# KohakuBlueleaf/UwUDiff

Measured on AMD Instinct MI355X. Metric: train images/sec (whole node), DiT-S/2 256^2 latent, higher is better.
Workload: dtype bf16; 1 GPU; DiT-S/2 (L12 D384 h6), 4x32x32 synthetic latents + pooled-text cond 1280, eps-MSE, AdamW lr1e-6 wd0.01 cosine; random-init weights; per_gpu_batch=768, global_batch=768, parallelism=dp1

## Files before the change

### uwudiff_amd/csrc/gemm_as.hip

```cpp
#include "gemm_shared.h"

namespace {

constexpr int AS_K = 384, AS_BN = 64, AS_STAGE = AS_BN * AS_K * 2;
constexpr int AS_NST = 3;
constexpr int AS_LDS = AS_NST * AS_STAGE + 8192;
template <typename TC, int EPI>
__global__ void __launch_bounds__(512, 2) gemm_as_kernel(const GemmArgs g) {
  extern __shared__ __attribute__((aligned(16))) char smem[];
  typedef bf16_t T;
  constexpr int FI = 2, FJ = 4, KS = AS_K / 32;
  const int tid = threadIdx.x, lane = tid & 63;
  const int wave = __builtin_amdgcn_readfirstlane(tid >> 6);
  const int fr = lane & 15, fq = lane >> 4;
  const int m0 = blockIdx.x * 256 + wave * 32;
  const T* A = static_cast<const T*>(g.A);
  const T* B = static_cast<const T*>(g.B);
  float* bias_lds = reinterpret_cast<float*>(smem + AS_NST * AS_STAGE);
  if (EPI == UWU_EPI_BIAS || EPI == UWU_EPI_BIAS_GELU)
    for (int n = tid; n < g.N; n += 512) bias_lds[n] = g.bias[n];

  uint4 af[FI][KS];
#pragma unroll
  for (int i = 0; i < FI; ++i)
#pragma unroll
    for (int s = 0; s < KS; ++s)
      af[i][s] = *reinterpret_cast<const uint4*>(A + (int64_t)(m0 + 16 * i + fr) * g.lda + 32 * s + 8 * fq);

  const int drow = 8 * wave + (lane >> 3);
  const int dc = ((lane & 7) ^ (drow >> 1) ^ (drow >> 4)) & 7;
  const T* bsrc = B + (int64_t)drow * g.ldb + 8 * dc;
  const unsigned smem_base = (unsigned)(size_t)((const __attribute__((address_space(3))) char*)smem);
  auto issue = [&](int c) {
    const T* p = bsrc + (int64_t)c * AS_BN * g.ldb;
#pragma unroll
    for (int q = 0; q < AS_K / 64; ++q)
      glds16_asm(p + 64 * q, smem_base + (unsigned)((c % AS_NST) * AS_STAGE + q * 8192 + wave * 1024));
  };
  const int nchunks = g.N / AS_BN;
  static_assert(EPI == UWU_EPI_BIAS_GELU || EPI == UWU_EPI_BIAS || EPI == UWU_EPI_DGELU, "the interleaved epilogues");
  constexpr int NS = EPI == UWU_EPI_BIAS ? 4 : 8;
  TC* const C = static_cast<TC*>(g.C);
  TC* const C2 = static_cast<TC*>(g.C2);
  const bool odd = fq & 1;
  auto pack = [](const f32x4& v) {
    bf16x4 b = {(bf16_t)v[0], (bf16_t)v[1], (bf16_t)v[2], (bf16_t)v[3]};
    return *reinterpret_cast<uint2*>(&b);
  };
  uint4 auxr[4];
  const T* const auxp = static_cast<const T*>(g.aux);
  auto aux_load = [&](int n0, int u) {
    const int i = u >> 1, jp = u & 1;
    const int m = m0 + 16 * i + fr, n = n0 + 32 * jp + (odd ? 16 + 4 * (fq - 1) : 4 * fq);
    auxr[u] = *reinterpret_cast<const uint4*>(auxp + (int64_t)m * g.ldaux + n);
  };
  auto epi_unit = [&](const f32x4 (&pa)[FI][FJ], int n0, int i, int jp) {
    f32x4 v0 = pa[i][2 * jp], v1 = pa[i][2 * jp + 1];
    typedef unsigned su32x2 __attribute__((ext_vector_type(2)));
    typedef unsigned su32x4 __attribute__((ext_vector_type(4)));
    if constexpr (EPI == UWU_EPI_DGELU) {
      const uint4 a = auxr[2 * i + jp];
      const su32x2 sx = __builtin_amdgcn_permlane16_swap(a.x, a.z, false, false);
      const su32x2 sy = __builtin_amdgcn_permlane16_swap(a.y, a.w, false, false);
      const uint2 r0 = {sx[0], sy[0]}, r1 = {sx[1], sy[1]};
      const bf16x4 u0 = *reinterpret_cast<const bf16x4*>(&r0), u1 = *reinterpret_cast<const bf16x4*>(&r1);
      v0 = v0 * dgelu_tanh_f4(f32x4{(float)u0[0], (float)u0[1], (float)u0[2], (float)u0[3]});
      v1 = v1 * dgelu_tanh_f4(f32x4{(float)u1[0], (float)u1[1], (float)u1[2], (float)u1[3]});
    } else {
      const float* bl = bias_lds + n0 + 32 * jp + 4 * fq;
      v0 = v0 + *reinterpret_cast<const f32x4*>(bl);
      v1 = v1 + *reinterpret_cast<const f32x4*>(bl + 16);
    }
    const int m = m0 + 16 * i + fr;
    const int n = n0 + 32 * jp + (odd ? 16 + 4 * (fq - 1) : 4 * fq);
    auto exchange_store = [&](TC* dst, const f32x4& x0, const f32x4& x1, bool stream_out) {
      const uint2 p0 = pack(x0), p1 = pack(x1);
      const su32x2 sx = __builtin_amdgcn_permlane16_swap(p0.x, p1.x, false, false);
      const su32x2 sy = __builtin_amdgcn_permlane16_swap(p0.y, p1.y, false, false);
      const su32x4 o = su32x4{sx[0], sy[0], sx[1], sy[1]};
      su32x4* ptr = reinterpret_cast<su32x4*>(dst + (int64_t)m * g.ldc + n);
      if (stream_out) __builtin_nontemporal_store(o, ptr);
      else *ptr = o;
    };
    if constexpr (EPI == UWU_EPI_BIAS_GELU) {
      exchange_store(C, v0, v1, true);
      exchange_store(C2, gelu_tanh_f4(v0), gelu_tanh_f4(v1), false);
    } else {
      exchange_store(C, v0, v1, false);
    }
  };
  f32x4 prev[FI][FJ];
#pragma unroll
  for (int i = 0; i < FI; ++i)
#pragma unroll
    for (int j = 0; j < FJ; ++j) prev[i][j] = f32x4{0.f, 0.f, 0.f, 0.f};
  issue(0);
  issue(1);
  for (int c = 0; c < nchunks; ++c) {
    if (c == 0) asm volatile("s_waitcnt vmcnt(6) lgkmcnt(0)" ::: "memory");
    else if (c <= 2 || c + 1 >= nchunks) asm volatile("s_waitcnt vmcnt(0)" ::: "memory");
    else asm volatile("s_waitcnt vmcnt(%0)" ::"n"(2 * NS + 6) : "memory");
    __builtin_amdgcn_s_barrier();
    if (c + 2 < nchunks) issue(c + 2);
    const char* lb = smem + (c % AS_NST) * AS_STAGE;
    f32x4 acc[FI][FJ];
#pragma unroll
    for (int i = 0; i < FI; ++i)
#pragma unroll
      for (int j = 0; j < FJ; ++j) acc[i][j] = f32x4{0.f, 0.f, 0.f, 0.f};
    constexpr int NBF = EPI == UWU_EPI_DGELU ? 1 : 2;
    uint4 bf[NBF][FJ];
    auto frags = [&](uint4 (&dst)[FJ], int s) {
#pragma unroll
      for (int j = 0; j < FJ; ++j)
        dst[j] = *reinterpret_cast<const uint4*>(lb + (s >> 1) * 8192 + swz(16 * j + fr, 4 * (s & 1) + fq));
    };
    if constexpr (NBF == 2) frags(bf[0], 0);
#pragma unroll
    for (int s = 0; s < KS; ++s) {
      if constexpr (NBF == 2) {
        if (s + 1 < KS) frags(bf[(s + 1) & 1], s + 1);
      } else {
        frags(bf[0], s);
      }
#pragma unroll
      for (int i = 0; i < FI; ++i)
#pragma unroll
        for (int j = 0; j < FJ; ++j) mma_frag<T>(bf[s & (NBF - 1)][j], af[i][s], acc[i][j]);
      if (s % 3 == 1) {
        if (c > 0) epi_unit(prev, (c - 1) * AS_BN, (s / 3) >> 1, (s / 3) & 1);
        if constexpr (EPI == UWU_EPI_DGELU) aux_load(c * AS_BN, s / 3);
      }
    }
#pragma unroll
    for (int i = 0; i < FI; ++i)
#pragma unroll
      for (int j = 0; j < FJ; ++j) prev[i][j] = acc[i][j];
  }
#pragma unroll
  for (int u = 0; u < 4; ++u) epi_unit(prev, (nchunks - 1) * AS_BN, u >> 1, u & 1);
}

}

bool uwu_gemm_use_as(const GemmArgs& g, int out_bytes) {
  static UwuEnv on("UWU_GEMM_AS");
  if (on.get().is('0')) return false;
  return g.K == AS_K && g.M % 256 == 0 && g.M >= 256 * 256 && g.N % AS_BN == 0 && g.N <= 2048 && g.N >= 1024 && out_bytes == 2 &&
         g.lda % 8 == 0 &&
         g.ldb % 8 == 0 && g.ldc % 8 == 0 && (((uintptr_t)g.A | (uintptr_t)g.B | (uintptr_t)g.C | (uintptr_t)g.C2) & 15) == 0;
}
bool uwu_gemm_use_as_bias() {
  static UwuEnv on("UWU_GEMM_AS_BIAS");
  return !on.get().is('0');
}


template <typename TC, int EPI>
int uwu_launch_gemm_as(GemmArgs g, hipStream_t st) {
  g.wide = 1;
  return gemm_launch<gemm_as_kernel<TC, EPI>>("gemm_as", AS_LDS, dim3(g.M / 256), 512, st, gemm_prof(g, false, sizeof(TC)), g);
}

template int uwu_launch_gemm_as<bf16_t, UWU_EPI_BIAS>(GemmArgs, hipStream_t);
template int uwu_launch_gemm_as<bf16_t, UWU_EPI_BIAS_GELU>(GemmArgs, hipStream_t);
template int uwu_launch_gemm_as<bf16_t, UWU_EPI_DGELU>(GemmArgs, hipStream_t);
```

### uwudiff_amd/csrc/gemm_shared.h

```cpp
#pragma once
#include <stdlib.h>

#include <atomic>
#include <type_traits>

#include "common.h"

#define RETURN_IF(...)             \
  do {                             \
    const int rc_ = (__VA_ARGS__); \
    if (rc_ != UWU_OK) return rc_; \
  } while (0)

extern std::atomic<const char*> g_uwu_gemm_last_kernel;

struct GemmArgs {
  const void* A;
  const void* B;
  void* C;
  void* C2;
  const float* bias;
  const void* aux;
  int M, N, K, lda, ldb, ldc, ldaux, epi, tiles_m, tiles_n, k_tiles_per_split, wide;
  int xs, nloc, part_m;
  int aux16;
  int cH, cW, cC, cHo, cWo, cS;
  const void* zero;
  void* q8;
  void* q8t;
  const float* q_scale;
  float* q_amax;
  int ldq, ldqt;
};

namespace {

constexpr int BM = 128, BN = 128;
constexpr int ROW_BYTES = 128;
constexpr int TILE_BYTES = 128 * ROW_BYTES;

template <typename T> struct GT;
template <> struct GT<bf16_t> { static constexpr int EPC = 8; static constexpr int BK = 64; };
template <> struct GT<float> { static constexpr int EPC = 4; static constexpr int BK = 32; };

__device__ __forceinline__ int swz(int row, int chunk) {
  return row * ROW_BYTES + (((chunk ^ (row >> 1) ^ (row >> 4)) & 7) << 4);
}

typedef unsigned gu32x4 __attribute__((ext_vector_type(4)));
__device__ __forceinline__ uint4 lds_read128_asm(const char* p) {
  gu32x4 v;
  const unsigned a = (unsigned)(size_t)((const __attribute__((address_space(3))) char*)p);
  asm volatile("ds_read_b128 %0, %1" : "=v"(v) : "v"(a) : "memory");
  return uint4{v[0], v[1], v[2], v[3]};
}

template <typename T, bool TRANS>
struct Stager {
  uint4 r[4];

  __device__ __forceinline__ void load(const T* __restrict__ base, int ld, int row0, int k0, int nrows, int K,
                                       int tid) {
    constexpr int EPC = GT<T>::EPC;
    if constexpr (!TRANS) {
      const int c = tid & 7, rr = tid >> 3;
      const int kk = k0 + c * EPC;
#pragma unroll
      for (int p = 0; p < 4; ++p) {
        const int grow = row0 + rr + 32 * p;
        if (grow < nrows && kk < K)
          r[p] = *reinterpret_cast<const uint4*>(base + (int64_t)grow * ld + kk);
        else
          r[p] = uint4{0, 0, 0, 0};
      }
    } else if constexpr (sizeof(T) == 2) {
      const int xg = tid & 15, kg = tid >> 4;
      const int x = row0 + 8 * xg;
#pragma unroll
      for (int kr = 0; kr < 4; ++kr) {
        const int k = k0 + 4 * kg + kr;
        if (k < K && x < nrows)
          r[kr] = *reinterpret_cast<const uint4*>(base + (int64_t)k * ld + x);
        else
          r[kr] = uint4{0, 0, 0, 0};
      }
    } else {
      const int xg = tid & 31, kg = tid >> 5;
      const int x = row0 + 4 * xg;
#pragma unroll
      for (int kr = 0; kr < 4; ++kr) {
        const int k = k0 + 4 * kg + kr;
        if (k < K && x < nrows)
          r[kr] = *reinterpret_cast<const uint4*>(base + (int64_t)k * ld + x);
        else
          r[kr] = uint4{0, 0, 0, 0};
      }
    }
  }

  __device__ __forceinline__ void store(char* __restrict__ lds, int tid) const {
    if constexpr (!TRANS) {
      const int c = tid & 7, rr = tid >> 3;
#pragma unroll
      for (int p = 0; p < 4; ++p) *reinterpret_cast<uint4*>(lds + swz(rr + 32 * p, c)) = r[p];
    } else if constexpr (sizeof(T) == 2) {
      const int xg = tid & 15, kg = tid >> 4;
      const unsigned* w0 = reinterpret_cast<const unsigned*>(&r[0]);
      const unsigned* w1 = reinterpret_cast<const unsigned*>(&r[1]);
      const unsigned* w2 = reinterpret_cast<const unsigned*>(&r[2]);
      const unsigned* w3 = reinterpret_cast<const unsigned*>(&r[3]);
#pragma unroll
      for (int xi = 0; xi < 8; ++xi) {
        const int row = 8 * xg + xi;
        const unsigned sel = (xi & 1) ? 0x07060302u : 0x05040100u;
        uint2 o;
        o.x = __builtin_amdgcn_perm(w1[xi >> 1], w0[xi >> 1], sel);
        o.y = __builtin_amdgcn_perm(w3[xi >> 1], w2[xi >> 1], sel);
        *reinterpret_cast<uint2*>(lds + swz(row, kg >> 1) + 8 * (kg & 1)) = o;
      }
    } else {
      const int xg = tid & 31, kg = tid >> 5;
      const unsigned* w0 = reinterpret_cast<const unsigned*>(&r[0]);
      const unsigned* w1 = reinterpret_cast<const unsigned*>(&r[1]);
      const unsigned* w2 = reinterpret_cast<const unsigned*>(&r[2]);
      const unsigned* w3 = reinterpret_cast<const unsigned*>(&r[3]);
#pragma unroll
      for (int xi = 0; xi < 4; ++xi) {
        const int row = 4 * xg + xi;
        *reinterpret_cast<uint4*>(lds + swz(row, kg)) = uint4{w0[xi], w1[xi], w2[xi], w3[xi]};
      }
    }
  }
};

template <typename T>
__device__ __forceinline__ void glds_tile(const T* __restrict__ base, int ld, int row0, int k0, int nrows,
                                          char* __restrict__ lds_tile, int tid) {
  constexpr int EPC = GT<T>::EPC;
  const int wave = tid >> 6, lane = tid & 63;
#pragma unroll
  for (int g = 0; g < 4; ++g) {
    const int grp = wave + 4 * g;
    const int row = 8 * grp + (lane >> 3);
    const int c = ((lane & 7) ^ (row >> 1) ^ (row >> 4)) & 7;
    int grow = row0 + row;
    if (grow >= nrows) grow = nrows - 1;
    const T* src = base + (int64_t)grow * ld + k0 + c * EPC;
    __builtin_amdgcn_global_load_lds((const __attribute__((address_space(1))) void*)src,
                                     (__attribute__((address_space(3))) void*)(lds_tile + grp * 1024), 16, 0, 0);
  }
}

template <typename T>
__device__ __forceinline__ void mma_frag(const uint4& a, const uint4& b, f32x4& c) {
  if constexpr (sizeof(T) == 2) {
    c = __builtin_amdgcn_mfma_f32_16x16x32_bf16(*reinterpret_cast<const bf16x8*>(&a),
                                                *reinterpret_cast<const bf16x8*>(&b), c, 0, 0, 0);
  } else {
    const float* af = reinterpret_cast<const float*>(&a);
    const float* bf = reinterpret_cast<const float*>(&b);
#pragma unroll
    for (int e = 0; e < 4; ++e) c = __builtin_amdgcn_mfma_f32_16x16x4f32(af[e], bf[e], c, 0, 0, 0);
  }
}



__device__ __forceinline__ void divmod24(int n, int d, float rcp, int& q, int& r) {
  q = (int)((float)n * rcp);
  r = n - q * d;
  if (r < 0) { r += d; --q; }
  if (r >= d) { r -= d; ++q; }
}

template <typename T, int FI, int FJ>
struct EpiPre {
  static constexpr int PD = FI < 4 ? FI : 4;
  typedef typename std::conditional<sizeof(T) == 2, uint2, f32x4>::type AuxRaw;
  f32x4 bias[FJ];
  AuxRaw aux[PD][FJ];
};
template <typename T, int FI, int FJ>
__device__ __forceinline__ void epi_load_aux_row(const GemmArgs& g, int m_w, int n_w, int fr, int fq, int i,
                                                 typename EpiPre<T, FI, FJ>::AuxRaw (&dst)[FJ]) {
  typedef typename EpiPre<T, FI, FJ>::AuxRaw AuxRaw;
  const T* aux = static_cast<const T*>(g.aux);
  const int m = m_w + 16 * i + fr;
  if constexpr (sizeof(T) == 2 && FJ % 2 == 0) {
    if (g.aux16) {
      const bool odd = fq & 1;
#pragma unroll
      for (int jp = 0; jp < FJ / 2; ++jp) {
        const int nb = n_w + 32 * jp;
        const int n = odd ? nb + 16 + 4 * (fq - 1) : nb + 4 * fq;
        uint4 v = {0u, 0u, 0u, 0u};
        if (m < g.M && n < g.N) v = *reinterpret_cast<const uint4*>(aux + (int64_t)m * g.ldaux + n);
        dst[2 * jp] = AuxRaw{v.x, v.y};
        dst[2 * jp + 1] = AuxRaw{v.z, v.w};
      }
      return;
    }
  }
#pragma unroll
  for (int j = 0; j < FJ; ++j) {
    const int n = n_w + 16 * j + 4 * fq;
    if (m < g.M && n < g.N) dst[j] = *reinterpret_cast<const AuxRaw*>(aux + (int64_t)m * g.ldaux + n);
    else dst[j] = AuxRaw{};
  }
}
template <typename T, int FI, int FJ, int EPI>
__device__ __forceinline__ void epi_prefetch(EpiPre<T, FI, FJ>& pre, const GemmArgs& g, int m_w, int n_w, int fr,
                                             int fq) {
  const int epi = EPI >= 0 ? EPI : g.epi;
  const bool has_bias = epi == UWU_EPI_BIAS || epi == UWU_EPI_BIAS_GELU || epi == UWU_EPI_BIAS_SILU;
#pragma unroll
  for (int j = 0; j < FJ; ++j) {
    const int n = n_w + 16 * j + 4 * fq;
    pre.bias[j] = (has_bias && n < g.N) ? load4(g.bias + n) : f32x4{0.f, 0.f, 0.f, 0.f};
  }
  if (epi == UWU_EPI_DGELU) {
#pragma unroll
    for (int i = 0; i < EpiPre<T, FI, FJ>::PD; ++i) epi_load_aux_row<T, FI, FJ>(g, m_w, n_w, fr, fq, i, pre.aux[i]);
  }
}

template <typename T, typename TC, int FI, int FJ, int EPI = -1>
__device__ __forceinline__ void epilogue_tile(f32x4 (&acc)[FI][FJ], EpiPre<T, FI, FJ>& pre, const GemmArgs& g, int m_w,
                                              int n_w, int fr, int fq, float* cs_lds, int wm, int wn, int cs_t = -1,
                                              f32x4* cs_out = nullptr) {
  TC* C = static_cast<TC*>(g.C);
  TC* C2 = static_cast<TC*>(g.C2);
  const int epi = EPI >= 0 ? EPI : g.epi;
  const bool has_bias = epi == UWU_EPI_BIAS || epi == UWU_EPI_BIAS_GELU || epi == UWU_EPI_BIAS_SILU;
  const bool two = epi == UWU_EPI_BIAS_GELU || epi == UWU_EPI_BIAS_SILU;
  const bool dgelu = epi == UWU_EPI_DGELU;
  constexpr int PD = EpiPre<T, FI, FJ>::PD;
  typedef typename EpiPre<T, FI, FJ>::AuxRaw AuxRaw;
  auto aux_f32 = [](const AuxRaw& r) {
    if constexpr (sizeof(T) == 2) {
      const bf16x4 b = *reinterpret_cast<const bf16x4*>(&r);
      return f32x4{(float)b[0], (float)b[1], (float)b[2], (float)b[3]};
    } else {
      return r;
    }
  };

  auto finish = [&](f32x4 v, const f32x4& b, const AuxRaw& a, f32x4& second) {
    if (has_bias) v = v + b;
    if (dgelu) {
      v = v * dgelu_tanh_f4(aux_f32(a));
    }
    if (epi == UWU_EPI_BIAS_GELU) {
      second = gelu_tanh_f4(v);
    } else if (epi == UWU_EPI_BIAS_SILU) {
#pragma unroll
      for (int e = 0; e < 4; ++e) second[e] = silu_f(v[e]);
    }
    return v;
  };
  float* colsum = dgelu ? reinterpret_cast<float*>(g.C2) : nullptr;
  f32x4 csum[FJ];
#pragma unroll
  for (int j = 0; j < FJ; ++j) csum[j] = f32x4{0.f, 0.f, 0.f, 0.f};
  auto add_cs = [&](f32x4& acc_, const f32x4& v) { acc_ = acc_ + v; };
  auto flush_cs = [&]() {
    if (!colsum) return;
    constexpr int BNT = 2 * 16 * FJ;
    __syncthreads();
#pragma unroll
    for (int j = 0; j < FJ; ++j) {
      f32x4 v = csum[j];
#pragma unroll
      for (int e = 0; e < 4; ++e) v[e] = row16_sum(v[e]);
      if (fr == 0) store4(cs_lds + wm * BNT + wn * 16 * FJ + 16 * j + 4 * fq, v);
    }
    __syncthreads();
    const int t = cs_t >= 0 ? cs_t : (int)threadIdx.x, n = n_w - wn * 16 * FJ + t;
    if (t < BNT && n < g.N) atomicAdd(colsum + n, cs_lds[t] + cs_lds[BNT + t]);
  };
  const bool wide = sizeof(TC) == 2 && g.wide;
  const bool odd = fq & 1;
  auto pack = [](const f32x4& v) {
    bf16x4 b = {(bf16_t)v[0], (bf16_t)v[1], (bf16_t)v[2], (bf16_t)v[3]};
    return *reinterpret_cast<uint2*>(&b);
  };
#pragma unroll
  for (int i = 0; i < FI; ++i) {
    const int m = m_w + 16 * i + fr;
    const bool mok = m < g.M;
    AuxRaw(&arow)[FJ] = pre.aux[i % PD];
    if constexpr (sizeof(T) == 2 && FJ % 2 == 0) {
      if (dgelu && g.aux16) {
#pragma unroll
        for (int jp = 0; jp < FJ / 2; ++jp) {
          typedef unsigned su32x2 __attribute__((ext_vector_type(2)));
          const su32x2 sx = __builtin_amdgcn_permlane16_swap(arow[2 * jp].x, arow[2 * jp + 1].x, false, false);
          const su32x2 sy = __builtin_amdgcn_permlane16_swap(arow[2 * jp].y, arow[2 * jp + 1].y, false, false);
          arow[2 * jp] = AuxRaw{sx[0], sy[0]};
          arow[2 * jp + 1] = AuxRaw{sx[1], sy[1]};
        }
      }
    }
    f32x4 v[FJ], sec[FJ];
#pragma unroll
    for (int j = 0; j < FJ; ++j) {
      const int n = n_w + 16 * j + 4 * fq;
      sec[j] = f32x4{0.f, 0.f, 0.f, 0.f};
      v[j] = (mok && n < g.N) ? finish(acc[i][j], pre.bias[j], arow[j], sec[j]) : acc[i][j];
      if (colsum && mok && n < g.N) add_cs(csum[j], v[j]);
    }
    if (dgelu && i + PD < FI) epi_load_aux_row<T, FI, FJ>(g, m_w, n_w, fr, fq, i + PD, arow);
    if (wide) {
      if constexpr (sizeof(TC) == 2) {
#pragma unroll
        for (int jp = 0; jp < FJ / 2; ++jp) {
          const int nb = n_w + 32 * jp;
          auto exchange_store = [&](TC* dst, const f32x4& x0, const f32x4& x1, bool stream_out = false) {
            const uint2 p0 = pack(x0), p1 = pack(x1);
            typedef unsigned su32x2 __attribute__((ext_vector_type(2)));
            const su32x2 sx = __builtin_amdgcn_permlane16_swap(p0.x, p1.x, false, false);
            const su32x2 sy = __builtin_amdgcn_permlane16_swap(p0.y, p1.y, false, false);
            const int n = odd ? nb + 16 + 4 * (fq - 1) : nb + 4 * fq;
            if (mok && n < g.N) {
              typedef unsigned su32x4 __attribute__((ext_vector_type(4)));
              const su32x4 o = su32x4{sx[0], sy[0], sx[1], sy[1]};
              su32x4* ptr = reinterpret_cast<su32x4*>(dst + (int64_t)m * g.ldc + n);
              if (stream_out) __builtin_nontemporal_store(o, ptr);
              else *ptr = o;
            }
          };
          exchange_store(C, v[2 * jp], v[2 * jp + 1], epi == UWU_EPI_BIAS_GELU);
          if (two) exchange_store(C2, sec[2 * jp], sec[2 * jp + 1], false);
        }
      }
    } else {
#pragma unroll
      for (int j = 0; j < FJ; ++j) {
        const int n = n_w + 16 * j + 4 * fq;
        if (!mok || n >= g.N) continue;
        store4(C + (int64_t)m * g.ldc + n, v[j]);
        if (two) store4(C2 + (int64_t)m * g.ldc + n, sec[j]);
      }
    }
  }
  if (cs_out) {
#pragma unroll
    for (int j = 0; j < FJ; ++j) cs_out[j] = cs_out[j] + csum[j];
  } else {
    flush_cs();
  }
}

constexpr int R_ROWB = 64;
constexpr int R_BSUB = 32 * 256;

__device__ __forceinline__ int r_gsw(int row) { return (0 - (row >> 2)) & 3; }
__device__ __forceinline__ int r_swz(int row, int chunk) { return row * R_ROWB + (((chunk ^ r_gsw(row)) & 3) << 4); }
template <int OFF>
__device__ __forceinline__ uint4 r_read128(unsigned addr) {
  gu32x4 v;
  asm volatile("ds_read_b128 %0, %1 offset:%2" : "=v"(v) : "v"(addr), "n"(OFF) : "memory");
  return uint4{v[0], v[1], v[2], v[3]};
}
template <int N>
__device__ __forceinline__ void r_wait_vm() {
  asm volatile("s_waitcnt vmcnt(%0)" ::"n"(N) : "memory");
}
__device__ __forceinline__ void glds16_asm(const void* gsrc, unsigned lds_dst ) {
  unsigned keep;
  asm volatile("s_mov_b32 %0, m0\n\ts_mov_b32 m0, %2\n\ts_nop 0\n\tglobal_load_lds_dwordx4 %1, off\n\ts_mov_b32 m0, %0"
               : "=&s"(keep)
               : "v"(gsrc), "s"(lds_dst)
               : "memory");
}
template <int H>
using IC = std::integral_constant<int, H>;
__device__ __forceinline__ int p8_swz(int row, int chunk) { return row * ROW_BYTES + (((chunk ^ (row >> 1)) & 7) << 4); }

template <int OFF>
__device__ __forceinline__ uint2 t_read_tr(unsigned addr) {
  typedef unsigned tu32x2 __attribute__((ext_vector_type(2)));
  tu32x2 v;
  asm volatile("ds_read_b64_tr_b16 %0, %1 offset:%2" : "=v"(v) : "v"(addr), "n"(OFF) : "memory");
  return uint2{v[0], v[1]};
}
__device__ __forceinline__ unsigned tr_lane_base(int lane, int t, int xb8) {
  const int tg = lane >> 4, tq = (lane >> 2) & 3, tp = lane & 3;
  const int krow = 8 * tg + 4 * t + tq;
  const int f = (tq << 2) | ((2 * tg + t) & 3);
  return (unsigned)(256 * krow + 16 * ((xb8 + (tp >> 1)) ^ f) + 8 * (tp & 1));
}

static int gemm_tag(const GemmArgs& g, bool tb, bool acc) {
  if (acc) return UWU_PROF_GEMM_WGRAD;
  if (g.epi == UWU_EPI_BIAS_GELU) return UWU_PROF_GEMM_FC1_GELU;
  if (g.epi == UWU_EPI_DGELU) return UWU_PROF_GEMM_FC2_DGELU;
  return tb ? UWU_PROF_GEMM_DGRAD : UWU_PROF_GEMM_FWD;
}
static double gemm_bytes(const GemmArgs& g, int es, int esc) {
  double b = ((double)g.M * g.K + (double)g.N * g.K) * es + (double)g.M * g.N * esc;
  if (g.epi == UWU_EPI_BIAS_GELU || g.epi == UWU_EPI_BIAS_SILU) b += (double)g.M * g.N * esc;
  if (g.epi == UWU_EPI_DGELU) b += (double)g.M * g.N * es;
  return b;
}

template <auto KERN>
int gemm_lds_optin(const char* name, int lds) {
  static unsigned char done[UWU_MAX_DEV];
  if (uwu_func_lds(reinterpret_cast<const void*>(KERN), lds, done)) return UWU_OK;
  uwu_set_error("%s: the device cannot give a workgroup %d bytes of LDS", name, lds);
  return UWU_ELAUNCH;
}
struct GemmProf {
  int tag, kind;
  double flops, bytes;
};
static GemmProf gemm_prof(const GemmArgs& g, bool tb, int esc) {
  return {gemm_tag(g, tb, false), 0, 2.0 * g.M * g.N * g.K, gemm_bytes(g, 2, esc)};
}
template <auto KERN, typename... Args>
int gemm_launch(const char* name, int lds, dim3 grid, int block, hipStream_t st, const GemmProf& p, const Args&... args) {
  RETURN_IF(gemm_lds_optin<KERN>(name, lds));
  g_uwu_gemm_last_kernel.store(name, std::memory_order_relaxed);
  UwuProfScope prof(st);
  hipLaunchKernelGGL(KERN, grid, dim3(block), lds, st, args...);
  prof.done(p.tag, p.kind, p.flops, p.bytes);
  UWU_LAUNCH_CHECK(name);
  return UWU_OK;
}

}

bool uwu_gemm_use_as(const GemmArgs& g, int out_bytes);
bool uwu_gemm_use_as_bias();
template <typename TC, int EPI> int uwu_launch_gemm_as(GemmArgs g, hipStream_t st);
int uwu_conv3x3_args(GemmArgs& g, int B, int H, int W, int C, int stride);
int uwu_gemm_pick_tr(const GemmArgs& g);
template <int FI, int FJ, bool CONVW = false> int uwu_launch_gemm_tr(GemmArgs g, void* scratch, size_t scratch_bytes, hipStream_t st);
void uwu_launch_splitk_reduce(const float* part, float* C, int M, int N, int ldc, int split, hipStream_t st);
int uwu_launch_gemm_p8(const GemmArgs& g, bool tb, hipStream_t st);
int uwu_p8_cus();
bool uwu_gemm_p8_ok(const GemmArgs& g, bool tb);
int uwu_launch_gemm_p8n(const GemmArgs& g, bool tb, hipStream_t st);
bool uwu_gemm_p8n_ok(const GemmArgs& g, bool tb);
bool uwu_gemm_p8f_ok(const GemmArgs& g);
int uwu_launch_gemm_p8f(GemmArgs g, int fmt_a, const float* sa, const float* sb, hipStream_t st);
int uwu_gemm_p8f_split(int tiles, int steps);
bool uwu_gemm_p8f_part_ok(const GemmArgs& g);
int uwu_launch_gemm_p8f_part(GemmArgs& g, int fmt_a, const float* sa, const float* sb, void* scratch, hipStream_t st);
```

Before: 17860 images/s.

## Split B-tile loads across two wave groups in the DGELU AS GEMM

```diff
diff --git a/uwudiff_amd/csrc/gemm_as.hip b/uwudiff_amd/csrc/gemm_as.hip
--- a/uwudiff_amd/csrc/gemm_as.hip
+++ b/uwudiff_amd/csrc/gemm_as.hip
@@ -5,7 +5,7 @@
 constexpr int AS_K = 384, AS_BN = 64, AS_STAGE = AS_BN * AS_K * 2;
 constexpr int AS_NST = 3;
 constexpr int AS_LDS = AS_NST * AS_STAGE + 8192;
-template <typename TC, int EPI>
+template <typename TC, int EPI, bool GRP>
 __global__ void __launch_bounds__(512, 2) gemm_as_kernel(const GemmArgs g) {
   extern __shared__ __attribute__((aligned(16))) char smem[];
   typedef bf16_t T;
@@ -31,11 +31,16 @@
   const int dc = ((lane & 7) ^ (drow >> 1) ^ (drow >> 4)) & 7;
   const T* bsrc = B + (int64_t)drow * g.ldb + 8 * dc;
   const unsigned smem_base = (unsigned)(size_t)((const __attribute__((address_space(3))) char*)smem);
+  const unsigned boff = (unsigned)(drow * g.ldb + 8 * dc) * 2;
   auto issue = [&](int c) {
     const T* p = bsrc + (int64_t)c * AS_BN * g.ldb;
-#pragma unroll
-    for (int q = 0; q < AS_K / 64; ++q)
-      glds16_asm(p + 64 * q, smem_base + (unsigned)((c % AS_NST) * AS_STAGE + q * 8192 + wave * 1024));
+    const T* ps = B + (int64_t)c * AS_BN * g.ldb;
+#pragma unroll
+    for (int q = 0; q < AS_K / 64; ++q) {
+      const unsigned dst = smem_base + (unsigned)((c % AS_NST) * AS_STAGE + q * 8192 + wave * 1024);
+      if constexpr (GRP) glds16_asm_s(ps + 64 * q, boff, dst);
+      else glds16_asm(p + 64 * q, dst);
+    }
   };
   const int nchunks = g.N / AS_BN;
   static_assert(EPI == UWU_EPI_BIAS_GELU || EPI == UWU_EPI_BIAS || EPI == UWU_EPI_DGELU, "the interleaved epilogues");
@@ -94,14 +99,33 @@
   for (int i = 0; i < FI; ++i)
 #pragma unroll
     for (int j = 0; j < FJ; ++j) prev[i][j] = f32x4{0.f, 0.f, 0.f, 0.f};
+  const int grp = GRP ? wave >> 2 : 0;
+  auto wait_chunk = [&](int w) __attribute__((always_inline)) {
+    if (w <= 2 || w + 1 >= nchunks) asm volatile("s_waitcnt vmcnt(0)" ::: "memory");
+    else asm volatile("s_waitcnt vmcnt(%0)" ::"n"(GRP ? 3 * NS / 2 + 6 : 2 * NS + 6) : "memory");
+  };
   issue(0);
   issue(1);
+  if (GRP && grp == 1) {
+    asm volatile("s_waitcnt vmcnt(6) lgkmcnt(0)" ::: "memory");
+    __builtin_amdgcn_s_barrier();
+  }
   for (int c = 0; c < nchunks; ++c) {
-    if (c == 0) asm volatile("s_waitcnt vmcnt(6) lgkmcnt(0)" ::: "memory");
-    else if (c <= 2 || c + 1 >= nchunks) asm volatile("s_waitcnt vmcnt(0)" ::: "memory");
-    else asm volatile("s_waitcnt vmcnt(%0)" ::"n"(2 * NS + 6) : "memory");
-    __builtin_amdgcn_s_barrier();
-    if (c + 2 < nchunks) issue(c + 2);
+    if constexpr (!GRP) {
+      if (c == 0) asm volatile("s_waitcnt vmcnt(6) lgkmcnt(0)" ::: "memory");
+      else wait_chunk(c);
+      __builtin_amdgcn_s_barrier();
+      if (c + 2 < nchunks) issue(c + 2);
+    } else {
+      asm volatile("s_waitcnt lgkmcnt(0)" ::: "memory");
+      if (grp == 0) {
+        if (c == 0) asm volatile("s_waitcnt vmcnt(6)" ::: "memory");
+        else wait_chunk(c);
+      }
+      __builtin_amdgcn_s_barrier();
+      __builtin_amdgcn_sched_barrier(0);
+      if (grp == 1 && c + 2 < nchunks) issue(c + 2);
+    }
     const char* lb = smem + (c % AS_NST) * AS_STAGE;
     f32x4 acc[FI][FJ];
 #pragma unroll
@@ -123,6 +147,14 @@
       } else {
         frags(bf[0], s);
       }
+      if constexpr (GRP) {
+        if (s == KS / 2) {
+          if (grp == 1 && c + 1 < nchunks) wait_chunk(c + 1);
+          __builtin_amdgcn_s_barrier();
+          __builtin_amdgcn_sched_barrier(0);
+          if (grp == 0 && c + 2 < nchunks) issue(c + 2);
+        }
+      }
 #pragma unroll
       for (int i = 0; i < FI; ++i)
 #pragma unroll
@@ -139,6 +171,7 @@
   }
 #pragma unroll
   for (int u = 0; u < 4; ++u) epi_unit(prev, (nchunks - 1) * AS_BN, u >> 1, u & 1);
+  if (GRP && grp == 0) __builtin_amdgcn_s_barrier();
 }
 
 }
@@ -158,8 +191,12 @@
 
 template <typename TC, int EPI>
 int uwu_launch_gemm_as(GemmArgs g, hipStream_t st) {
+  static UwuEnv groups("UWU_AS_GROUPS");
   g.wide = 1;
-  return gemm_launch<gemm_as_kernel<TC, EPI>>("gemm_as", AS_LDS, dim3(g.M / 256), 512, st, gemm_prof(g, false, sizeof(TC)), g);
+  constexpr bool grouped = EPI == UWU_EPI_DGELU;
+  if (!grouped || groups.get().is('0'))
+    return gemm_launch<gemm_as_kernel<TC, EPI, false>>("gemm_as", AS_LDS, dim3(g.M / 256), 512, st, gemm_prof(g, false, sizeof(TC)), g);
+  return gemm_launch<gemm_as_kernel<TC, EPI, grouped>>("gemm_as", AS_LDS, dim3(g.M / 256), 512, st, gemm_prof(g, false, sizeof(TC)), g);
 }
 
 template int uwu_launch_gemm_as<bf16_t, UWU_EPI_BIAS>(GemmArgs, hipStream_t);
diff --git a/uwudiff_amd/csrc/gemm_shared.h b/uwudiff_amd/csrc/gemm_shared.h
--- a/uwudiff_amd/csrc/gemm_shared.h
+++ b/uwudiff_amd/csrc/gemm_shared.h
@@ -373,6 +373,13 @@
                : "v"(gsrc), "s"(lds_dst)
                : "memory");
 }
+__device__ __forceinline__ void glds16_asm_s(const void* gbase , unsigned lane_off, unsigned lds_dst ) {
+  unsigned keep;
+  asm volatile("s_mov_b32 %0, m0\n\ts_mov_b32 m0, %3\n\ts_nop 0\n\tglobal_load_lds_dwordx4 %1, %2\n\ts_mov_b32 m0, %0"
+               : "=&s"(keep)
+               : "v"(lane_off), "s"(gbase), "s"(lds_dst)
+               : "memory");
+}
 template <int H>
 using IC = std::integral_constant<int, H>;
 __device__ __forceinline__ int p8_swz(int row, int chunk) { return row * ROW_BYTES + (((chunk ^ (row >> 1)) & 7) << 4); }
```

Measured after the change: 17900 images/s (median of 6 runs). About the same (+0.2%).
